# DataZooDE/anofox-statistics

Measured on AMD Instinct MI355X. Metric: group_fits_per_sec, higher is better.
Workload: dtype f64; 1 GPU; ols_fit_agg: 1000000 groups x n=1000 x p=8, device-resident grouped columns, fit_intercept=true, compute_inference=false; groups_total=1000000, groups_per_gpu=1000000, rows_per_group=1000, features=8, partition=contiguous key ranges over 1 rank(s); all-gather of 14-double records

## Files before the change

anofox-statistics_amd/csrc/accumulate_narrow.hip:

```cpp
#include <stdlib.h>

#include "common.h"
#include "wave_reduce.h"

namespace anofox {

typedef double dbl2u __attribute__((ext_vector_type(2), aligned(8)));

#ifndef ANOFOX_NARROW_NT
#define ANOFOX_NARROW_NT false
#endif
template <bool NT>
__device__ __forceinline__ dbl2u load2(const double *p) {
	if (NT) return __builtin_nontemporal_load(reinterpret_cast<const dbl2u *>(p));
	return *reinterpret_cast<const dbl2u *>(p);
}

template <int Z>
struct NarrowTile {
	double n0[Z], n1[Z], nw0, nw1;
};

template <int P, bool WEIGHTED>
__device__ __forceinline__ void narrow_load_tile(const BatchArgs &args, int64_t base, int64_t hi, int lane, NarrowTile<P + 1> &t) {
	const int64_t r0 = base + 2 * lane;
	if (base + 128 <= hi) {
#pragma unroll
		for (int j = 0; j < P; ++j) {
			const dbl2u v = load2<ANOFOX_NARROW_NT>(args.x[j] + r0);
			t.n0[j] = v.x;
			t.n1[j] = v.y;
		}
		{
			const dbl2u v = load2<ANOFOX_NARROW_NT>(args.y + r0);
			t.n0[P] = v.x;
			t.n1[P] = v.y;
		}
		if (WEIGHTED) {
			const dbl2u v = load2<ANOFOX_NARROW_NT>(args.w + r0);
			t.nw0 = v.x;
			t.nw1 = v.y;
		}
	} else {
		const int64_t c0 = r0 < hi ? r0 : hi - 1, c1 = r0 + 1 < hi ? r0 + 1 : hi - 1;
#pragma unroll
		for (int j = 0; j < P; ++j) {
			t.n0[j] = args.x[j][c0];
			t.n1[j] = args.x[j][c1];
		}
		t.n0[P] = args.y[c0];
		t.n1[P] = args.y[c1];
		if (WEIGHTED) {
			t.nw0 = args.w[c0];
			t.nw1 = args.w[c1];
// ... 114 lines not shown
	for (int k = 0; k < ZZ; ++k) v[L::OFF_Q + k] = c.q[k];
	v[L::OFF_SW] = c.sw;

	transpose_reduce64(v, lane);

	if (lane < L::KRED) rec[lane] = v[0];

	double e = 0.0;
#pragma unroll
	for (int a = 0; a < Z; ++a) e = (lane == a) ? c.first[a] : e;
	e = (lane == Z) ? (double)c.cnt : e;
	e = (lane == Z + 1) ? (double)c.mask : e;
	if (lane < Z + 2) rec[L::KRED + lane] = e;
}

template <int P, bool WEIGHTED, bool CENTER, bool PREFETCH>
__device__ __forceinline__ void accumulate_rows(const BatchArgs &args, int64_t lo, int64_t hi, double *rec, int lane) {
	constexpr int Z = P + 1;
	NarrowAcc<P> c;
	narrow_acc_init<P>(c);
	NarrowTile<Z> t;
	if (PREFETCH && lo < hi) narrow_load_tile<P, WEIGHTED>(args, lo, hi, lane, t);
	for (int64_t base = lo; base < hi; base += 128) {
		if (!PREFETCH) narrow_load_tile<P, WEIGHTED>(args, base, hi, lane, t);
		double z0[Z], z1[Z];
		double w0 = 1.0, w1 = 1.0;
#pragma unroll
		for (int a = 0; a < Z; ++a) {
			z0[a] = t.n0[a];
			z1[a] = t.n1[a];
		}
		if (WEIGHTED) {
			w0 = t.nw0;
			w1 = t.nw1;
		}
		if (PREFETCH && base + 128 < hi) narrow_load_tile<P, WEIGHTED>(args, base + 128, hi, lane, t);
		narrow_tile_compute<P, WEIGHTED, CENTER>(c, z0, z1, w0, w1, base + 2 * lane, hi);
	}
	narrow_acc_finish<P, CENTER>(c, rec, lane);
}

__device__ __forceinline__ SegHeader *seg_header(void *t) { return static_cast<SegHeader *>(t); }
__device__ __forceinline__ SegBigGroup *seg_big(void *t) { return reinterpret_cast<SegBigGroup *>(seg_header(t) + 1); }
__device__ __forceinline__ SegEntry *seg_entries(void *t) { return reinterpret_cast<SegEntry *>(seg_big(t) + kSegMaxBig); }
__device__ __forceinline__ double *seg_records(void *t) { return reinterpret_cast<double *>(seg_entries(t) + kSegMaxSegments); }

__device__ __forceinline__ bool narrow_register_big_group(const BatchArgs &args, int64_t g, int64_t lo, int64_t hi, int lane) {
	{
		SegHeader *h = seg_header(args.seg_table);
		const int64_t S = args.seg_rows;
		const int nseg = (int)((hi - lo + S - 1) / S);
// ... 21 lines not shown
			if (slot >= 0) return true;
		}
	}
	return false;
}

template <int P, bool WEIGHTED, bool CENTER, bool PF>
__device__ __forceinline__ void accumulate_group(const BatchArgs &args, int64_t g, int lane) {
	using L = MomentLayout<P>;
	const int64_t lo = args.row_offsets[g];
	const int64_t hi = group_row_end(args, g);
	if (args.seg_table && hi - lo > args.seg_rows && narrow_register_big_group(args, g, lo, hi, lane)) return;
	accumulate_rows<P, WEIGHTED, CENTER, PF>(args, lo, hi, args.moments + g * (int64_t)L::REC, lane);
}

template <int P, bool WEIGHTED, bool CENTER, bool PF>
__global__ __launch_bounds__(256) void accumulate_narrow_kernel(BatchArgs args) {
	const int lane = threadIdx.x & 63;
	const int64_t g = __builtin_amdgcn_readfirstlane((int)(threadIdx.x >> 6)) + (int64_t)blockIdx.x * 4;
	if (g >= args.n_groups) return;
	accumulate_group<P, WEIGHTED, CENTER, PF>(args, g, lane);
}

template <int P, bool WEIGHTED, bool CENTER, bool PF>
__global__ __launch_bounds__(256) void accumulate_narrow_list_kernel(BatchArgs args, const int32_t *list, const int32_t *count) {
	const int lane = threadIdx.x & 63;
	const int n = *count;
	const int n_waves = (int)gridDim.x * 4;
	for (int v = (int)blockIdx.x * 4 + __builtin_amdgcn_readfirstlane((int)(threadIdx.x >> 6)); v < n; v += n_waves)
		accumulate_group<P, WEIGHTED, CENTER, PF>(args, list[v], lane);
}

template <int P, bool CENTER>
__device__ void merge_segments(const double *seg_rec, int nseg, double *rec, int lane) {
// ... 54 lines not shown
	if (v >= total) return;
	const SegEntry e = seg_entries(args.seg_table)[v];
	if (e.slot < 0) return;
	double *recs = seg_records(args.seg_table);
	accumulate_rows<P, WEIGHTED, CENTER, PF>(args, e.lo, e.hi, recs + (int64_t)v * L::REC, lane);
	__threadfence();
	SegBigGroup *b = seg_big(args.seg_table) + e.slot;
	int old = 0;
	if (lane == 0) old = atomicAdd(&b->done, 1);
	old = __builtin_amdgcn_readfirstlane(old);
	if (old != b->nseg - 1) return;
	__threadfence();
	merge_segments<P, CENTER>(recs + (int64_t)b->base * L::REC, b->nseg, args.moments + b->g * (int64_t)L::REC, lane);
}

template <int P, bool PF>
static hipError_t launch_pn(const BatchArgs &a, hipStream_t stream) {
	const dim3 block(256);
	const dim3 grid((unsigned)((a.n_groups + 3) / 4));
	const dim3 seg_grid((unsigned)((kSegMaxSegments + 3) / 4));
	const bool weighted = a.model == ANOFOX_HIP_MODEL_WLS;
	const bool center = a.fit_intercept != 0;
#define ANOFOX_ACC_LAUNCH(W, C)                                                                               \
	do {                                                                                                      \
		hipLaunchKernelGGL((accumulate_narrow_kernel<P, W, C, PF>), grid, block, 0, stream, a);               \
		if (a.seg_table) hipLaunchKernelGGL((accumulate_segments_kernel<P, W, C, PF>), seg_grid, block, 0, stream, a); \
	} while (0)
	if (weighted) {
		if (center) ANOFOX_ACC_LAUNCH(true, true);
		else ANOFOX_ACC_LAUNCH(true, false);
	} else {
		if (center) ANOFOX_ACC_LAUNCH(false, true);
		else ANOFOX_ACC_LAUNCH(false, false);
	}
#undef ANOFOX_ACC_LAUNCH
	return hipGetLastError();
}

template <int P, bool PF>
static hipError_t launch_list_pn(const BatchArgs &a, const int32_t *list, const int32_t *count, hipStream_t stream) {
	const dim3 block(256), grid(2048);
	const dim3 seg_grid((unsigned)((kSegMaxSegments + 3) / 4));
	const bool weighted = a.model == ANOFOX_HIP_MODEL_WLS;
	const bool center = a.fit_intercept != 0;
#define ANOFOX_ACC_LIST_LAUNCH(W, C)                                                                          \
	do {                                                                                                      \
		hipLaunchKernelGGL((accumulate_narrow_list_kernel<P, W, C, PF>), grid, block, 0, stream, a, list, count); \
		if (a.seg_table) hipLaunchKernelGGL((accumulate_segments_kernel<P, W, C, PF>), seg_grid, block, 0, stream, a); \
	} while (0)
	if (weighted) {
		if (center) ANOFOX_ACC_LIST_LAUNCH(true, true);
		else ANOFOX_ACC_LIST_LAUNCH(true, false);
	} else {
		if (center) ANOFOX_ACC_LIST_LAUNCH(false, true);
		else ANOFOX_ACC_LIST_LAUNCH(false, false);
	}
#undef ANOFOX_ACC_LIST_LAUNCH
	return hipGetLastError();
}

template <int P>
static hipError_t launch_p(const BatchArgs &a, const int32_t *list, const int32_t *count, hipStream_t stream) {
	static const int pf = [] { const char *e = getenv("ANOFOX_ACC_PF"); return e ? atoi(e) : 1; }();
	if (list) return pf ? launch_list_pn<P, true>(a, list, count, stream) : launch_list_pn<P, false>(a, list, count, stream);
	return pf ? launch_pn<P, true>(a, stream) : launch_pn<P, false>(a, stream);
}

static hipError_t launch_any(const BatchArgs &a, const int32_t *list, const int32_t *count, hipStream_t stream) {
	if (a.n_groups <= 0) return hipSuccess;
	switch (a.p) {
	case 1: return launch_p<1>(a, list, count, stream);
	case 2: return launch_p<2>(a, list, count, stream);
	case 3: return launch_p<3>(a, list, count, stream);
	case 4: return launch_p<4>(a, list, count, stream);
	case 5: return launch_p<5>(a, list, count, stream);
	case 6: return launch_p<6>(a, list, count, stream);
	case 7: return launch_p<7>(a, list, count, stream);
	case 8: return launch_p<8>(a, list, count, stream);
	default: return hipErrorInvalidValue;
	}
}

hipError_t launch_accumulate_narrow(const BatchArgs &a, hipStream_t stream) { return launch_any(a, nullptr, nullptr, stream); }

hipError_t launch_accumulate_narrow_list(const BatchArgs &a, const int32_t *list, const int32_t *count, hipStream_t stream) {
	return launch_any(a, list, count, stream);
}

}
```

anofox-statistics_amd/csrc/common.h:

```cpp
#pragma once
#include <hip/hip_runtime.h>
#include <stdint.h>

#include "../../include/anofox_stats_hip.h"

namespace anofox {

constexpr int kNarrowMaxP = 8;

constexpr size_t kTcritTableBytes = 4096;

template <int P>
struct MomentLayout {
	static constexpr int Z = P + 1;
	static constexpr int ZZ = Z * (Z + 1) / 2;
	static constexpr int OFF_S = 0;
	static constexpr int OFF_Q = Z;
	static constexpr int OFF_SW = Z + ZZ;
	static constexpr int KRED = Z + ZZ + 1;
	static constexpr int OFF_FIRST = KRED;
	static constexpr int OFF_CNT = KRED + Z;
	static constexpr int OFF_MASK = KRED + Z + 1;
	static constexpr int REC = KRED + Z + 2;
	__host__ __device__ static constexpr int q_index(int a, int b) {
// ... 29 lines not shown
	int lambda_scaling;
	int hc_type;
	double confidence_level;
	double alpha;
	double *moments;
	double *core;
	double *inference;
	int32_t *refine_list;
	int32_t *refine_count;
	double *refine_vec;
	void *tcrit_table;
	const int64_t *rule_counts;
	void *seg_table;
	int64_t seg_rows;
	const int64_t *row_ends;
};
inline __host__ __device__ int64_t group_row_end(const BatchArgs &a, int64_t g) { return a.row_ends ? a.row_ends[g] : a.row_offsets[g + 1]; }

constexpr int kSegTargetWaves = 2048;
constexpr int kSegMaxBig = kSegTargetWaves + 8;
constexpr int kSegMaxSegments = 2 * kSegTargetWaves + 16;
constexpr int64_t kSegMinRows = 8192;
struct SegHeader {
	int32_t seg_total;
	int32_t big_total;
	int32_t pad[14];
};
struct SegBigGroup {
	int64_t g;
	int32_t base;
	int32_t nseg;
// ... 384 lines not shown
```

anofox-statistics_amd/csrc/host_api.hip:

```cpp
#include <math.h>
#include <stdio.h>
#include <stdlib.h>
#include <string.h>

#include <memory>
#include <mutex>
#include <string>
#include <vector>

#include "common.h"
#include "host_math.h"

using namespace anofox;

#include "context.h"

using namespace anofox::host;

namespace {

struct Workspace {
	void *seg_table;
	double *moments;
	double *refine_vec;
// ... 35 lines not shown
	}
	if (hip_fail(launch_residual_grad_wide(a, ss), "wide residual kernel launch", e)) return false;
	if (hip_fail(solve(2), "wide final kernel launch", e)) return false;
	if (!mid && hip_fail(launch_inference_wide_finish(a, ss), "wide inference finish kernel launch", e)) return false;
	if (a.hc_type != ANOFOX_HC_NONE && a.inference && a.model != ANOFOX_HIP_MODEL_RIDGE) {
		if (!ensure_buffer(&ctx->aux, &ctx->aux_bytes, (size_t)slab * sizeof(double), "hc scratch", e)) return false;
		a.hc_df = (double *)ctx->aux;
		if (hip_fail(launch_hc_wide(a, ss), "wide hc kernel launch", e)) return false;
	}
	static const bool refit_dd_on = !(getenv("ANOFOX_REFIT_DD") && atoi(getenv("ANOFOX_REFIT_DD")) == 0);
	if (refit_dd_on && hip_fail(launch_refit_dd_wide(a, ss), "double-double refit kernel launch", e)) return false;
	return true;
}

bool regression_narrow_stage(AnofoxHipContext *ctx, BatchArgs &a, hipStream_t st, void *, AnofoxError *e) {
	if (hip_fail(launch_solve_narrow(a, st), "solve kernel launch", e)) return false;
	if (hip_fail(launch_refine_fused_narrow(a, kRefineSteps, st), "refine kernel launch", e)) return false;
	if (a.hc_type != ANOFOX_HC_NONE && a.inference && a.model != ANOFOX_HIP_MODEL_RIDGE) {
		const size_t b_tab = align_up(sizeof(PredictSegTable), 256);
		if (!ensure_buffer(&ctx->aux, &ctx->aux_bytes, b_tab + hc_prep_bytes(a.n_groups, a.p), "hc scratch", e)) return false;
		if (hip_fail(hipMemsetAsync(ctx->aux, 0, 64, st), "hipMemsetAsync", e)) return false;
		if (hip_fail(launch_hc_narrow(a, (double *)((char *)ctx->aux + b_tab), ctx->aux, st), "hc kernel launch", e)) return false;
	}
	static const bool refit_dd_on = !(getenv("ANOFOX_REFIT_DD") && atoi(getenv("ANOFOX_REFIT_DD")) == 0);
	if (refit_dd_on && hip_fail(launch_refit_dd_narrow(a, st), "double-double refit kernel launch", e)) return false;
	return true;
}

const SolveStages kRegressionStages = {regression_narrow_stage, regression_wide_stage, nullptr};

bool run_wide_batch(AnofoxHipContext *ctx, int64_t G, size_t p, int64_t n_rows, const int64_t *d_off,
// ... 185 lines not shown
	hipEvent_t e0 = nullptr, e1 = nullptr, e2 = nullptr;
	if (ctx->timing) {
		e0 = get_event(ctx);
		e1 = get_event(ctx);
		e2 = get_event(ctx);
		(void)hipEventRecord(e0, st);
	}
	if (ctx->gate_wait) {
		hipEvent_t gw = ctx->gate_wait;
		ctx->gate_wait = nullptr;
		if (hip_fail(hipStreamWaitEvent(st, gw, 0), "hipStreamWaitEvent", e)) return false;
	}
	if (ctx->timing) (void)hipEventRecord(e0, st);
	static const bool small_on = !(getenv("ANOFOX_ACC_SMALL") && atoi(getenv("ANOFOX_ACC_SMALL")) == 0);
	const int segw = (small_on && !a.row_ends && n_rows > 0 && G < (int64_t)0x7fffffff) ? accumulate_small_segment_width((double)n_rows / (double)G) : 0;
	if (segw) {
		int32_t *big_count = ws.refine_count + 4;
		if (hip_fail(launch_accumulate_small(a, segw, ws.refine_list, big_count, st), "accumulate kernel launch", e)) return false;
		if (hip_fail(launch_accumulate_narrow_list(a, ws.refine_list, big_count, st), "accumulate kernel launch", e)) return false;
	} else if (hip_fail(launch_accumulate_narrow(a, st), "accumulate kernel launch", e)) {
		return false;
	}
	if (ctx->timing) (void)hipEventRecord(e1, st);
	if (ctx->gate_record) {
		hipEvent_t gr = ctx->gate_record;
		ctx->gate_record = nullptr;
		if (hip_fail(hipEventRecord(gr, st), "hipEventRecord", e)) return false;
	}
	if (!stages.narrow(ctx, a, st, stages.user, e)) return false;
	if (ctx->timing) {
// ... 1694 lines not shown
```

anofox-statistics_amd/csrc/solve_narrow.hip:

```cpp
#include "common.h"
#include "device_math.h"
#include "dd_arith.h"

namespace anofox {

static_assert(sizeof(TcritSlot) * kTcritSlots == kTcritTableBytes, "t memo does not fill its workspace slice");

namespace {

constexpr double kAliasTol = 1e-11;
constexpr double kAliasBand = 1e-13;
constexpr double kRefineTol = 1e-7;
constexpr double kPivotWarn = 1e-3;

__device__ __forceinline__ double nan64() { return __builtin_nan(""); }

enum { MODE_PRIMARY = 0, MODE_UPDATE = 1, MODE_FINAL = 2 };

template <int P, int MODE>
__device__ void solve_one(const BatchArgs &args, int64_t g) {
	using L = MomentLayout<P>;
	constexpr int Z = L::Z;
	const int p = P;
	const bool icpt = args.fit_intercept != 0;
	const int model = args.model;

	double *core = args.core + g * (int64_t)(p + 6);
	double *inf = (args.inference && args.compute_inference) ? args.inference + g * (int64_t)(5 * p + 2) : nullptr;
	const double *rv = args.refine_vec + g * (int64_t)refine_vec_len(p);

	int status = ANOFOX_ERROR_SUCCESS;
	double coef[P];
	double se[P], tv[P], pv[P], cl[P], cu[P];
#pragma unroll
	for (int j = 0; j < P; ++j) coef[j] = se[j] = tv[j] = pv[j] = cl[j] = cu[j] = nan64();
	double intercept = nan64(), r2 = nan64(), adj = nan64(), rse = nan64(), fstat = nan64(), fp = nan64();
	double nobs = nan64();
	bool has_inf = false;
	bool refine = false;

	const double *rec = args.moments + g * (int64_t)L::REC;
	const int64_t nrows = args.rule_counts ? args.rule_counts[g] : args.row_offsets[g + 1] - args.row_offsets[g];

	do {
		if (nrows < 2) { status = ANOFOX_HIP_STATUS_NULL_TOO_FEW_ROWS; break; }
		if (model == ANOFOX_HIP_MODEL_RIDGE && args.alpha < 0.0) { status = ANOFOX_ERROR_INVALID_ALPHA; break; }
		const double cnt = rec[L::OFF_CNT];
		if (!(cnt > 0.0)) { status = ANOFOX_ERROR_NO_VALID_DATA; break; }
		const double sw = rec[L::OFF_SW];
		const unsigned mask = (unsigned)rec[L::OFF_MASK];
		const int p_eff = __popc(mask);

		double s[Z], first[Z];
#pragma unroll
		for (int a = 0; a < Z; ++a) { s[a] = rec[L::OFF_S + a]; first[a] = rec[L::OFF_FIRST + a]; }
		const double qyy = rec[L::q_index(P, P)];
		const double cyy_centred = qyy - s[P] * s[P] / sw;
		const double ymean = (icpt ? first[P] : 0.0) + s[P] / sw;

		if (p_eff == 0) {
			if (!icpt) { status = ANOFOX_ERROR_INSUFFICIENT_DATA; break; }
			intercept = ymean;
			r2 = 0.0;
			adj = 0.0;
			rse = (model == ANOFOX_HIP_MODEL_WLS) ? sqrt(cyy_centred / sw) : sqrt(cyy_centred / (cnt - 1.0));
			nobs = cnt;
			break;
		}
		if (cnt < (double)(p_eff + (icpt ? 1 : 0))) { status = ANOFOX_ERROR_INSUFFICIENT_DATA; break; }

		double A[P][P];
		double c[P];
		bool active[P];
#pragma unroll
		for (int i = 0; i < P; ++i) {
			active[i] = (mask >> i) & 1u;
#pragma unroll
			for (int j = 0; j <= i; ++j) {
				const double qij = rec[L::q_index(j, i)];
				A[i][j] = icpt ? qij - s[i] * s[j] / sw : qij;
			}
			const double qiy = rec[L::q_index(i, P)];
			c[i] = icpt ? qiy - s[i] * s[P] / sw : qiy;
		}
		const double tss = icpt ? cyy_centred : qyy;

		double lam = 0.0, lam_rows = 0.0;
		bool glmnet_cancels = false;
		if (model == ANOFOX_HIP_MODEL_RIDGE) {
			lam = args.alpha;
			if (args.lambda_scaling == ANOFOX_LAMBDA_SCALING_GLMNET) {
				lam = cnt * args.alpha / sqrt(cyy_centred / cnt);
				glmnet_cancels = !icpt && !(cyy_centred * kGlmnetCancelRatio > qyy);
				if (MODE != MODE_PRIMARY && !icpt) lam_rows = cnt * args.alpha / sqrt(rv[p + 2] / cnt);
				else lam_rows = lam;
			} else {
				lam_rows = lam;
			}
#pragma unroll
			for (int i = 0; i < P; ++i) A[i][i] += (MODE == MODE_PRIMARY) ? lam : lam_rows;
		}

		double diag0[P];
#pragma unroll
		for (int j = 0; j < P; ++j) diag0[j] = A[j][j];
		double min_ratio = 1.0;
		bool band = false;
#pragma unroll
		for (int j = 0; j < P; ++j) {
			double d = A[j][j];
#pragma unroll
			for (int k = 0; k < j; ++k) d -= A[j][k] * A[j][k];
			const bool ok = active[j] && (d > kAliasTol * diag0[j]) && (d > 0.0);
			band = band || (active[j] && !ok && d > kAliasBand * diag0[j]);
			active[j] = ok;
			if (ok) min_ratio = fmin(min_ratio, d / diag0[j]);
			const double ljj = ok ? sqrt(d) : 1.0;
			A[j][j] = ljj;
			const double inv = 1.0 / ljj;
#pragma unroll
			for (int i = j + 1; i < P; ++i) {
				double t = A[i][j];
#pragma unroll
				for (int k = 0; k < j; ++k) t -= A[i][k] * A[j][k];
				A[i][j] = ok ? t * inv : 0.0;
			}
			if (!ok) {
#pragma unroll
				for (int k = 0; k < j; ++k) A[j][k] = 0.0;
			}
		}
		int rank = 0;
#pragma unroll
		for (int j = 0; j < P; ++j) rank += active[j] ? 1 : 0;

		auto solve_llt = [&](const double (&rhs)[P], double (&zf)[P], double (&x)[P]) {
#pragma unroll
			for (int i = 0; i < P; ++i) {
				double t = rhs[i];
#pragma unroll
				for (int k = 0; k < i; ++k) t -= A[i][k] * zf[k];
				zf[i] = active[i] ? t / A[i][i] : 0.0;
			}
#pragma unroll
			for (int i = P - 1; i >= 0; --i) {
				double t = zf[i];
#pragma unroll
				for (int k = i + 1; k < P; ++k) t -= A[k][i] * x[k];
				x[i] = active[i] ? t / A[i][i] : 0.0;
			}
		};

		double beta[P];
		double rss;
		if (MODE == MODE_PRIMARY) {
			double zf[P];
			solve_llt(c, zf, beta);
			double zz = 0.0, bc = 0.0, bb = 0.0;
#pragma unroll
			for (int i = 0; i < P; ++i) { zz += zf[i] * zf[i]; bc += beta[i] * c[i]; bb += beta[i] * beta[i]; }
			rss = (model == ANOFOX_HIP_MODEL_RIDGE) ? tss - bc - lam * bb : tss - zz;
			refine = !(rss > kRefineTol * tss) || (min_ratio < kPivotWarn) || glmnet_cancels || band;
			double bmax = 0.0;
#pragma unroll
			for (int i = 0; i < P; ++i) bmax = fmax(bmax, active[i] ? fabs(beta[i]) : 0.0);
#pragma unroll
			for (int i = 0; i < P; ++i) refine = refine || (active[i] && coef_bound_weak(beta[i], bmax, diag0[i], tss, min_ratio));
		} else {
#pragma unroll
			for (int i = 0; i < P; ++i) {
				const double b = core[i];
				beta[i] = active[i] ? b : 0.0;
			}
			rss = rv[0];
		}

		if (MODE == MODE_UPDATE) {
			const double gs = rv[1];
			double gc[P], u[P], delta[P];
#pragma unroll
			for (int i = 0; i < P; ++i) {
				double gi = rv[2 + i];
				if (icpt) gi -= (s[i] / sw) * gs;
				gc[i] = active[i] ? gi - lam_rows * beta[i] : 0.0;
			}
			solve_llt(gc, u, delta);
#pragma unroll
			for (int i = 0; i < P; ++i) beta[i] += delta[i];
		}

		const int n_par = rank + (icpt ? 1 : 0);
		const double df = cnt - (double)n_par;
		const double dfm = (double)rank;

		double b0 = 0.0;
		if (icpt) {
			b0 = ymean;
#pragma unroll
			for (int i = 0; i < P; ++i) b0 -= beta[i] * (first[i] + s[i] / sw);
			intercept = b0;
		}
#pragma unroll
		for (int i = 0; i < P; ++i) coef[i] = active[i] ? beta[i] : nan64();
		if (MODE == MODE_UPDATE) {
#pragma unroll
			for (int j = 0; j < P; ++j) core[j] = coef[j];
			core[p] = intercept;
			return;
		}
		r2 = 1.0 - rss / tss;
		adj = 1.0 - (1.0 - r2) * (cnt - (icpt ? 1.0 : 0.0)) / df;
		rse = sqrt(rss / df);
		nobs = cnt;
		fstat = ((tss - rss) / dfm) / (rss / df);

		if (inf) {
			has_inf = true;
			fp = dm_f_sf(fstat, dfm, df);
			const double sigma2 = rss / df;
			const double tcrit = dm_tcrit_cached(static_cast<TcritSlot *>(args.tcrit_table), 0.5 * (1.0 + args.confidence_level), df);
#pragma unroll
			for (int j = 0; j < P; ++j) {
				double wcol[P];
				double dj = 0.0;
#pragma unroll
				for (int i = j; i < P; ++i) {
					double t = (i == j) ? 1.0 : 0.0;
#pragma unroll
					for (int k = j; k < i; ++k) t -= A[i][k] * wcol[k];
					wcol[i] = active[i] ? t / A[i][i] : 0.0;
					dj += wcol[i] * wcol[i];
				}
				if (active[j]) {
					se[j] = sqrt(sigma2 * dj);
					tv[j] = beta[j] / se[j];
					pv[j] = dm_t_two_sided_p(tv[j], df);
					cl[j] = beta[j] - tcrit * se[j];
					cu[j] = beta[j] + tcrit * se[j];
				}
			}
		}
	} while (false);

	if (MODE == MODE_UPDATE) return;

	if (status != ANOFOX_ERROR_SUCCESS) {
#pragma unroll
		for (int j = 0; j < P; ++j) coef[j] = nan64();
		intercept = r2 = adj = rse = nobs = nan64();
	}
#pragma unroll
	for (int j = 0; j < P; ++j) core[j] = coef[j];
	core[p] = intercept;
	core[p + 1] = r2;
	core[p + 2] = adj;
	core[p + 3] = rse;
	core[p + 4] = nobs;
	core[p + 5] = (double)status;
	if (inf) {
		if (!has_inf) {
#pragma unroll
			for (int j = 0; j < P; ++j) se[j] = tv[j] = pv[j] = cl[j] = cu[j] = nan64();
			fstat = fp = nan64();
		}
#pragma unroll
		for (int j = 0; j < P; ++j) {
			inf[j] = se[j];
			inf[p + j] = tv[j];
			inf[2 * p + j] = pv[j];
			inf[3 * p + j] = cl[j];
			inf[4 * p + j] = cu[j];
		}
		inf[5 * p] = fstat;
		inf[5 * p + 1] = fp;
	}
	if (MODE == MODE_PRIMARY && refine && status == ANOFOX_ERROR_SUCCESS) {
		const int slot = atomicAdd(args.refine_count, 1);
		args.refine_list[slot] = (int32_t)g;
	}
}

template <int P>
__global__ __launch_bounds__(64) void solve_narrow_kernel(BatchArgs args) {
	const int64_t g = (int64_t)blockIdx.x * blockDim.x + threadIdx.x;
	if (g >= args.n_groups) return;
	solve_one<P, MODE_PRIMARY>(args, g);
}

__device__ __forceinline__ void residual_grad_wave(const BatchArgs &args, int64_t g, int lane) {
#pragma clang fp contract(off)
	const int p = args.p;
	const bool weighted = args.model == ANOFOX_HIP_MODEL_WLS;
	const int Z = p + 1;
	const int off_first = Z + Z * (Z + 1) / 2 + 1;
	const int rec_len = moment_record_len(p);
	const double *core = args.core + g * (int64_t)(p + 6);
	const double *rec = args.moments + g * (int64_t)rec_len;
	double b[kNarrowMaxP], sh[kNarrowMaxP], acc_h[kNarrowMaxP + 1], acc_l[kNarrowMaxP + 1];
	const double ybar = rec[p] / rec[Z + Z * (Z + 1) / 2] + (args.fit_intercept ? rec[off_first + p] : 0.0);
#pragma unroll
	for (int j = 0; j < kNarrowMaxP; ++j) {
// ... 53 lines not shown
	for (int k = 0; k < kNarrowMaxP + 1; ++k) mine = (lane == 1 + k) ? acc_h[k] + acc_l[k] : mine;
	if (lane == p + 2) mine = cyy;
	if (lane < p + 3) out[lane] = mine;
}

template <int P>
__global__ __launch_bounds__(64) void refine_fused_kernel(BatchArgs args, int steps) {
	const int lane = threadIdx.x & 63;
	const int n = *args.refine_count;
	for (int i = blockIdx.x; i < n; i += gridDim.x) {
		const int64_t g = args.refine_list[i];
		for (int it = 0; it <= steps; ++it) {
			residual_grad_wave(args, g, lane);
			__builtin_amdgcn_fence(__ATOMIC_SEQ_CST, "workgroup");
			if (lane == 0) {
				if (it < steps) solve_one<P, MODE_UPDATE>(args, g);
				else solve_one<P, MODE_FINAL>(args, g);
			}
			__builtin_amdgcn_fence(__ATOMIC_SEQ_CST, "workgroup");
		}
	}
}

template <int P>
hipError_t launch_solve_p(const BatchArgs &a, hipStream_t stream) {
	const unsigned grid = (unsigned)((a.n_groups + 63) / 64);
	hipLaunchKernelGGL((solve_narrow_kernel<P>), dim3(grid), dim3(64), 0, stream, a);
	return hipGetLastError();
}

}

// ... 39 lines not shown
```

Before: 80.60 million fits/s.

## Fuse narrow accumulation with primary solve, keeping moment records in LDS

Each wavefront now accumulates moments for up to 16 consecutive groups into shared memory. It then solves them in the same kernel, one lane per group, and writes only the core results plus the moments of groups queued for refinement. This removes the separate solve kernel launch and the global write and read of every group's moment record. Big segmented groups get a small dedicated solve kernel. The solve code moves into a shared header, and an env switch lets non-temporal loads be chosen at runtime. The tradeoff is that the serial per-lane solve runs inside the bandwidth-bound kernel, and the LDS use may cut occupancy.

```diff
diff --git a/anofox-statistics_amd/csrc/accumulate_narrow.hip b/anofox-statistics_amd/csrc/accumulate_narrow.hip
--- a/anofox-statistics_amd/csrc/accumulate_narrow.hip
+++ b/anofox-statistics_amd/csrc/accumulate_narrow.hip
@@ -1,15 +1,13 @@
 #include <stdlib.h>
 
 #include "common.h"
+#include "solve_narrow_impl.h"
 #include "wave_reduce.h"
 
 namespace anofox {
 
 typedef double dbl2u __attribute__((ext_vector_type(2), aligned(8)));
 
-#ifndef ANOFOX_NARROW_NT
-#define ANOFOX_NARROW_NT false
-#endif
 template <bool NT>
 __device__ __forceinline__ dbl2u load2(const double *p) {
 	if (NT) return __builtin_nontemporal_load(reinterpret_cast<const dbl2u *>(p));
@@ -21,23 +19,23 @@
 	double n0[Z], n1[Z], nw0, nw1;
 };
 
-template <int P, bool WEIGHTED>
+template <int P, bool WEIGHTED, bool NT>
 __device__ __forceinline__ void narrow_load_tile(const BatchArgs &args, int64_t base, int64_t hi, int lane, NarrowTile<P + 1> &t) {
 	const int64_t r0 = base + 2 * lane;
 	if (base + 128 <= hi) {
 #pragma unroll
 		for (int j = 0; j < P; ++j) {
-			const dbl2u v = load2<ANOFOX_NARROW_NT>(args.x[j] + r0);
+			const dbl2u v = load2<NT>(args.x[j] + r0);
 			t.n0[j] = v.x;
 			t.n1[j] = v.y;
 		}
 		{
-			const dbl2u v = load2<ANOFOX_NARROW_NT>(args.y + r0);
+			const dbl2u v = load2<NT>(args.y + r0);
 			t.n0[P] = v.x;
 			t.n1[P] = v.y;
 		}
 		if (WEIGHTED) {
-			const dbl2u v = load2<ANOFOX_NARROW_NT>(args.w + r0);
+			const dbl2u v = load2<NT>(args.w + r0);
 			t.nw0 = v.x;
 			t.nw1 = v.y;
 		}
@@ -182,15 +180,15 @@
 	if (lane < Z + 2) rec[L::KRED + lane] = e;
 }
 
-template <int P, bool WEIGHTED, bool CENTER, bool PREFETCH>
+template <int P, bool WEIGHTED, bool CENTER, bool PREFETCH, bool NT = false>
 __device__ __forceinline__ void accumulate_rows(const BatchArgs &args, int64_t lo, int64_t hi, double *rec, int lane) {
 	constexpr int Z = P + 1;
 	NarrowAcc<P> c;
 	narrow_acc_init<P>(c);
 	NarrowTile<Z> t;
-	if (PREFETCH && lo < hi) narrow_load_tile<P, WEIGHTED>(args, lo, hi, lane, t);
+	if (PREFETCH && lo < hi) narrow_load_tile<P, WEIGHTED, NT>(args, lo, hi, lane, t);
 	for (int64_t base = lo; base < hi; base += 128) {
-		if (!PREFETCH) narrow_load_tile<P, WEIGHTED>(args, base, hi, lane, t);
+		if (!PREFETCH) narrow_load_tile<P, WEIGHTED, NT>(args, base, hi, lane, t);
 		double z0[Z], z1[Z];
 		double w0 = 1.0, w1 = 1.0;
 #pragma unroll
@@ -202,7 +200,7 @@
 			w0 = t.nw0;
 			w1 = t.nw1;
 		}
-		if (PREFETCH && base + 128 < hi) narrow_load_tile<P, WEIGHTED>(args, base + 128, hi, lane, t);
+		if (PREFETCH && base + 128 < hi) narrow_load_tile<P, WEIGHTED, NT>(args, base + 128, hi, lane, t);
 		narrow_tile_compute<P, WEIGHTED, CENTER>(c, z0, z1, w0, w1, base + 2 * lane, hi);
 	}
 	narrow_acc_finish<P, CENTER>(c, rec, lane);
@@ -254,10 +252,55 @@
 	accumulate_rows<P, WEIGHTED, CENTER, PF>(args, lo, hi, args.moments + g * (int64_t)L::REC, lane);
 }
 
-template <int P, bool WEIGHTED, bool CENTER, bool PF>
-__global__ __launch_bounds__(256) void accumulate_narrow_kernel(BatchArgs args) {
+#ifndef ANOFOX_NARROW_FUSED_K
+#define ANOFOX_NARROW_FUSED_K 16
+#endif
+constexpr int kFusedGroups = ANOFOX_NARROW_FUSED_K;
+static_assert(kFusedGroups >= 1 && kFusedGroups <= 32, "groups per wavefront: one lane each, a 32-bit skip mask");
+
+template <int P, bool WEIGHTED, bool CENTER, bool PF, bool NT>
+__device__ __forceinline__ void accumulate_solve_groups(const BatchArgs &args, int64_t g0, int lane, double *lrec, double *lcore) {
+	using L = MomentLayout<P>;
+	constexpr int CL = P + 6;
+	const int n = (int)(args.n_groups - g0 < kFusedGroups ? args.n_groups - g0 : kFusedGroups);
+	unsigned skip = 0;
+	for (int i = 0; i < n; ++i) {
+		const int64_t g = g0 + i;
+		const int64_t lo = args.row_offsets[g];
+		const int64_t hi = group_row_end(args, g);
+		if (args.seg_table && hi - lo > args.seg_rows && narrow_register_big_group(args, g, lo, hi, lane)) {
+			skip |= 1u << i;
+			continue;
+		}
+		accumulate_rows<P, WEIGHTED, CENTER, PF, NT>(args, lo, hi, lrec + i * L::REC, lane);
+	}
+	__builtin_amdgcn_fence(__ATOMIC_SEQ_CST, "workgroup");
+	bool queued = false;
+	if (lane < n && !((skip >> lane) & 1u)) queued = solve_one<P, MODE_PRIMARY, false>(args, g0 + lane, lrec + lane * L::REC, lcore + lane * CL);
+	__builtin_amdgcn_fence(__ATOMIC_SEQ_CST, "workgroup");
+	double *core = args.core + g0 * CL;
+	for (int k = lane; k < n * CL; k += 64)
+		if (!((skip >> (k / CL)) & 1u)) core[k] = lcore[k];
+	for (unsigned long long q = __ballot(queued); q != 0ull; q &= q - 1ull) {
+		const int i = __ffsll((long long)q) - 1;
+		for (int k = lane; k < L::REC; k += 64) args.moments[(g0 + i) * L::REC + k] = lrec[i * L::REC + k];
+	}
+}
+
+template <int P, bool WEIGHTED, bool CENTER, bool PF, bool FUSED = false, bool NT = false>
+__global__ __launch_bounds__(256) __attribute__((amdgpu_waves_per_eu(FUSED ? 2 : 1))) void accumulate_narrow_kernel(BatchArgs args) {
 	const int lane = threadIdx.x & 63;
-	const int64_t g = __builtin_amdgcn_readfirstlane((int)(threadIdx.x >> 6)) + (int64_t)blockIdx.x * 4;
+	const int wave = __builtin_amdgcn_readfirstlane((int)(threadIdx.x >> 6));
+	if (FUSED) {
+		using L = MomentLayout<P>;
+		__shared__ double lrec[4][kFusedGroups * L::REC];
+		__shared__ double lcore[4][kFusedGroups * (P + 6)];
+		const int64_t g0 = ((int64_t)blockIdx.x * 4 + wave) * kFusedGroups;
+		if (g0 >= args.n_groups) return;
+		accumulate_solve_groups<P, WEIGHTED, CENTER, PF, NT>(args, g0, lane, lrec[wave], lcore[wave]);
+		return;
+	}
+	const int64_t g = wave + (int64_t)blockIdx.x * 4;
 	if (g >= args.n_groups) return;
 	accumulate_group<P, WEIGHTED, CENTER, PF>(args, g, lane);
 }
@@ -342,16 +385,28 @@
 	merge_segments<P, CENTER>(recs + (int64_t)b->base * L::REC, b->nseg, args.moments + b->g * (int64_t)L::REC, lane);
 }
 
-template <int P, bool PF>
+template <int P>
+__global__ __launch_bounds__(64) void solve_big_narrow_kernel(BatchArgs args) {
+	const int slot = (int)(blockIdx.x * blockDim.x + threadIdx.x);
+	const int total = seg_header(args.seg_table)->big_total;
+	if (slot >= total) return;
+	const int64_t g = seg_big(args.seg_table)[slot].g;
+	solve_one<P, MODE_PRIMARY>(args, g, args.moments + g * (int64_t)MomentLayout<P>::REC, args.core + g * (int64_t)(P + 6));
+}
+
+template <int P, bool PF, bool FUSED, bool NT>
 static hipError_t launch_pn(const BatchArgs &a, hipStream_t stream) {
 	const dim3 block(256);
-	const dim3 grid((unsigned)((a.n_groups + 3) / 4));
+	const int64_t per_block = FUSED ? 4 * kFusedGroups : 4;
+	const dim3 grid((unsigned)((a.n_groups + per_block - 1) / per_block));
 	const dim3 seg_grid((unsigned)((kSegMaxSegments + 3) / 4));
 	const bool weighted = a.model == ANOFOX_HIP_MODEL_WLS;
 	const bool center = a.fit_intercept != 0;
 #define ANOFOX_ACC_LAUNCH(W, C)                                                                               \
 	do {                                                                                                      \
-		hipLaunchKernelGGL((accumulate_narrow_kernel<P, W, C, PF>), grid, block, 0, stream, a);               \
+		constexpr bool F = FUSED && narrow_fused_fits(P, W, C);                                                      \
+		if (FUSED && !F) return hipErrorNotSupported;                                                         \
+		hipLaunchKernelGGL((accumulate_narrow_kernel<P, W, C, PF, F, F && NT>), grid, block, 0, stream, a);   \
 		if (a.seg_table) hipLaunchKernelGGL((accumulate_segments_kernel<P, W, C, PF>), seg_grid, block, 0, stream, a); \
 	} while (0)
 	if (weighted) {
@@ -362,6 +417,8 @@
 		else ANOFOX_ACC_LAUNCH(false, false);
 	}
 #undef ANOFOX_ACC_LAUNCH
+	if (FUSED && a.seg_table)
+		hipLaunchKernelGGL((solve_big_narrow_kernel<P>), dim3((unsigned)((kSegMaxBig + 63) / 64)), dim3(64), 0, stream, a);
 	return hipGetLastError();
 }
 
@@ -388,31 +445,36 @@
 }
 
 template <int P>
-static hipError_t launch_p(const BatchArgs &a, const int32_t *list, const int32_t *count, hipStream_t stream) {
+static hipError_t launch_p(const BatchArgs &a, const int32_t *list, const int32_t *count, bool fused, hipStream_t stream) {
 	static const int pf = [] { const char *e = getenv("ANOFOX_ACC_PF"); return e ? atoi(e) : 1; }();
+	static const int nt = [] { const char *e = getenv("ANOFOX_NARROW_NT"); return e ? atoi(e) : 0; }();
 	if (list) return pf ? launch_list_pn<P, true>(a, list, count, stream) : launch_list_pn<P, false>(a, list, count, stream);
-	return pf ? launch_pn<P, true>(a, stream) : launch_pn<P, false>(a, stream);
-}
-
-static hipError_t launch_any(const BatchArgs &a, const int32_t *list, const int32_t *count, hipStream_t stream) {
+	if (fused) {
+		if (!pf) return launch_pn<P, false, true, false>(a, stream);
+		return nt ? launch_pn<P, true, true, true>(a, stream) : launch_pn<P, true, true, false>(a, stream);
+	}
+	return pf ? launch_pn<P, true, false, false>(a, stream) : launch_pn<P, false, false, false>(a, stream);
+}
+
+static hipError_t launch_any(const BatchArgs &a, const int32_t *list, const int32_t *count, bool fused, hipStream_t stream) {
 	if (a.n_groups <= 0) return hipSuccess;
 	switch (a.p) {
-	case 1: return launch_p<1>(a, list, count, stream);
-	case 2: return launch_p<2>(a, list, count, stream);
-	case 3: return launch_p<3>(a, list, count, stream);
-	case 4: return launch_p<4>(a, list, count, stream);
-	case 5: return launch_p<5>(a, list, count, stream);
-	case 6: return launch_p<6>(a, list, count, stream);
-	case 7: return launch_p<7>(a, list, count, stream);
-	case 8: return launch_p<8>(a, list, count, stream);
+	case 1: return launch_p<1>(a, list, count, fused, stream);
+	case 2: return launch_p<2>(a, list, count, fused, stream);
+	case 3: return launch_p<3>(a, list, count, fused, stream);
+	case 4: return launch_p<4>(a, list, count, fused, stream);
+	case 5: return launch_p<5>(a, list, count, fused, stream);
+	case 6: return launch_p<6>(a, list, count, fused, stream);
+	case 7: return launch_p<7>(a, list, count, fused, stream);
+	case 8: return launch_p<8>(a, list, count, fused, stream);
 	default: return hipErrorInvalidValue;
 	}
 }
 
-hipError_t launch_accumulate_narrow(const BatchArgs &a, hipStream_t stream) { return launch_any(a, nullptr, nullptr, stream); }
+hipError_t launch_accumulate_narrow(const BatchArgs &a, hipStream_t stream) { return launch_any(a, nullptr, nullptr, a.primary_solved != 0, stream); }
 
 hipError_t launch_accumulate_narrow_list(const BatchArgs &a, const int32_t *list, const int32_t *count, hipStream_t stream) {
-	return launch_any(a, list, count, stream);
-}
-
-}
+	return launch_any(a, list, count, false, stream);
+}
+
+}
diff --git a/anofox-statistics_amd/csrc/common.h b/anofox-statistics_amd/csrc/common.h
--- a/anofox-statistics_amd/csrc/common.h
+++ b/anofox-statistics_amd/csrc/common.h
@@ -67,7 +67,11 @@
 	void *seg_table;
 	int64_t seg_rows;
 	const int64_t *row_ends;
-};
+	int primary_solved;
+};
+inline constexpr __host__ __device__ bool narrow_fused_fits(int p, bool weighted, bool center) {
+	return p >= 1 && p <= kNarrowMaxP && !(p == 8 && weighted && center);
+}
 inline __host__ __device__ int64_t group_row_end(const BatchArgs &a, int64_t g) { return a.row_ends ? a.row_ends[g] : a.row_offsets[g + 1]; }
 
 constexpr int kSegTargetWaves = 2048;
diff --git a/anofox-statistics_amd/csrc/host_api.hip b/anofox-statistics_amd/csrc/host_api.hip
--- a/anofox-statistics_amd/csrc/host_api.hip
+++ b/anofox-statistics_amd/csrc/host_api.hip
@@ -73,7 +73,7 @@
 }
 
 bool regression_narrow_stage(AnofoxHipContext *ctx, BatchArgs &a, hipStream_t st, void *, AnofoxError *e) {
-	if (hip_fail(launch_solve_narrow(a, st), "solve kernel launch", e)) return false;
+	if (!a.primary_solved && hip_fail(launch_solve_narrow(a, st), "solve kernel launch", e)) return false;
 	if (hip_fail(launch_refine_fused_narrow(a, kRefineSteps, st), "refine kernel launch", e)) return false;
 	if (a.hc_type != ANOFOX_HC_NONE && a.inference && a.model != ANOFOX_HIP_MODEL_RIDGE) {
 		const size_t b_tab = align_up(sizeof(PredictSegTable), 256);
@@ -289,6 +289,9 @@
 	if (ctx->timing) (void)hipEventRecord(e0, st);
 	static const bool small_on = !(getenv("ANOFOX_ACC_SMALL") && atoi(getenv("ANOFOX_ACC_SMALL")) == 0);
 	const int segw = (small_on && !a.row_ends && n_rows > 0 && G < (int64_t)0x7fffffff) ? accumulate_small_segment_width((double)n_rows / (double)G) : 0;
+	static const bool fused_on = !(getenv("ANOFOX_NARROW_FUSED") && atoi(getenv("ANOFOX_NARROW_FUSED")) == 0);
+	a.primary_solved = (fused_on && stages.narrow == regression_narrow_stage && !a.row_ends && !segw && !a.inference &&
+	                    narrow_fused_fits(a.p, a.model == ANOFOX_HIP_MODEL_WLS, a.fit_intercept != 0)) ? 1 : 0;
 	if (segw) {
 		int32_t *big_count = ws.refine_count + 4;
 		if (hip_fail(launch_accumulate_small(a, segw, ws.refine_list, big_count, st), "accumulate kernel launch", e)) return false;
diff --git a/anofox-statistics_amd/csrc/solve_narrow.hip b/anofox-statistics_amd/csrc/solve_narrow.hip
--- a/anofox-statistics_amd/csrc/solve_narrow.hip
+++ b/anofox-statistics_amd/csrc/solve_narrow.hip
@@ -1,6 +1,7 @@
 #include "common.h"
 #include "device_math.h"
 #include "dd_arith.h"
+#include "solve_narrow_impl.h"
 
 namespace anofox {
 
@@ -8,283 +9,11 @@
 
 namespace {
 
-constexpr double kAliasTol = 1e-11;
-constexpr double kAliasBand = 1e-13;
-constexpr double kRefineTol = 1e-7;
-constexpr double kPivotWarn = 1e-3;
-
-__device__ __forceinline__ double nan64() { return __builtin_nan(""); }
-
-enum { MODE_PRIMARY = 0, MODE_UPDATE = 1, MODE_FINAL = 2 };
-
-template <int P, int MODE>
-__device__ void solve_one(const BatchArgs &args, int64_t g) {
-	using L = MomentLayout<P>;
-	constexpr int Z = L::Z;
-	const int p = P;
-	const bool icpt = args.fit_intercept != 0;
-	const int model = args.model;
-
-	double *core = args.core + g * (int64_t)(p + 6);
-	double *inf = (args.inference && args.compute_inference) ? args.inference + g * (int64_t)(5 * p + 2) : nullptr;
-	const double *rv = args.refine_vec + g * (int64_t)refine_vec_len(p);
-
-	int status = ANOFOX_ERROR_SUCCESS;
-	double coef[P];
-	double se[P], tv[P], pv[P], cl[P], cu[P];
-#pragma unroll
-	for (int j = 0; j < P; ++j) coef[j] = se[j] = tv[j] = pv[j] = cl[j] = cu[j] = nan64();
-	double intercept = nan64(), r2 = nan64(), adj = nan64(), rse = nan64(), fstat = nan64(), fp = nan64();
-	double nobs = nan64();
-	bool has_inf = false;
-	bool refine = false;
-
-	const double *rec = args.moments + g * (int64_t)L::REC;
-	const int64_t nrows = args.rule_counts ? args.rule_counts[g] : args.row_offsets[g + 1] - args.row_offsets[g];
-
-	do {
-		if (nrows < 2) { status = ANOFOX_HIP_STATUS_NULL_TOO_FEW_ROWS; break; }
-		if (model == ANOFOX_HIP_MODEL_RIDGE && args.alpha < 0.0) { status = ANOFOX_ERROR_INVALID_ALPHA; break; }
-		const double cnt = rec[L::OFF_CNT];
-		if (!(cnt > 0.0)) { status = ANOFOX_ERROR_NO_VALID_DATA; break; }
-		const double sw = rec[L::OFF_SW];
-		const unsigned mask = (unsigned)rec[L::OFF_MASK];
-		const int p_eff = __popc(mask);
-
-		double s[Z], first[Z];
-#pragma unroll
-		for (int a = 0; a < Z; ++a) { s[a] = rec[L::OFF_S + a]; first[a] = rec[L::OFF_FIRST + a]; }
-		const double qyy = rec[L::q_index(P, P)];
-		const double cyy_centred = qyy - s[P] * s[P] / sw;
-		const double ymean = (icpt ? first[P] : 0.0) + s[P] / sw;
-
-		if (p_eff == 0) {
-			if (!icpt) { status = ANOFOX_ERROR_INSUFFICIENT_DATA; break; }
-			intercept = ymean;
-			r2 = 0.0;
-			adj = 0.0;
-			rse = (model == ANOFOX_HIP_MODEL_WLS) ? sqrt(cyy_centred / sw) : sqrt(cyy_centred / (cnt - 1.0));
-			nobs = cnt;
-			break;
-		}
-		if (cnt < (double)(p_eff + (icpt ? 1 : 0))) { status = ANOFOX_ERROR_INSUFFICIENT_DATA; break; }
-
-		double A[P][P];
-		double c[P];
-		bool active[P];
-#pragma unroll
-		for (int i = 0; i < P; ++i) {
-			active[i] = (mask >> i) & 1u;
-#pragma unroll
-			for (int j = 0; j <= i; ++j) {
-				const double qij = rec[L::q_index(j, i)];
-				A[i][j] = icpt ? qij - s[i] * s[j] / sw : qij;
-			}
-			const double qiy = rec[L::q_index(i, P)];
-			c[i] = icpt ? qiy - s[i] * s[P] / sw : qiy;
-		}
-		const double tss = icpt ? cyy_centred : qyy;
-
-		double lam = 0.0, lam_rows = 0.0;
-		bool glmnet_cancels = false;
-		if (model == ANOFOX_HIP_MODEL_RIDGE) {
-			lam = args.alpha;
-			if (args.lambda_scaling == ANOFOX_LAMBDA_SCALING_GLMNET) {
-				lam = cnt * args.alpha / sqrt(cyy_centred / cnt);
-				glmnet_cancels = !icpt && !(cyy_centred * kGlmnetCancelRatio > qyy);
-				if (MODE != MODE_PRIMARY && !icpt) lam_rows = cnt * args.alpha / sqrt(rv[p + 2] / cnt);
-				else lam_rows = lam;
-			} else {
-				lam_rows = lam;
-			}
-#pragma unroll
-			for (int i = 0; i < P; ++i) A[i][i] += (MODE == MODE_PRIMARY) ? lam : lam_rows;
-		}
-
-		double diag0[P];
-#pragma unroll
-		for (int j = 0; j < P; ++j) diag0[j] = A[j][j];
-		double min_ratio = 1.0;
-		bool band = false;
-#pragma unroll
-		for (int j = 0; j < P; ++j) {
-			double d = A[j][j];
-#pragma unroll
-			for (int k = 0; k < j; ++k) d -= A[j][k] * A[j][k];
-			const bool ok = active[j] && (d > kAliasTol * diag0[j]) && (d > 0.0);
-			band = band || (active[j] && !ok && d > kAliasBand * diag0[j]);
-			active[j] = ok;
-			if (ok) min_ratio = fmin(min_ratio, d / diag0[j]);
-			const double ljj = ok ? sqrt(d) : 1.0;
-			A[j][j] = ljj;
-			const double inv = 1.0 / ljj;
-#pragma unroll
-			for (int i = j + 1; i < P; ++i) {
-				double t = A[i][j];
-#pragma unroll
-				for (int k = 0; k < j; ++k) t -= A[i][k] * A[j][k];
-				A[i][j] = ok ? t * inv : 0.0;
-			}
-			if (!ok) {
-#pragma unroll
-				for (int k = 0; k < j; ++k) A[j][k] = 0.0;
-			}
-		}
-		int rank = 0;
-#pragma unroll
-		for (int j = 0; j < P; ++j) rank += active[j] ? 1 : 0;
-
-		auto solve_llt = [&](const double (&rhs)[P], double (&zf)[P], double (&x)[P]) {
-#pragma unroll
-			for (int i = 0; i < P; ++i) {
-				double t = rhs[i];
-#pragma unroll
-				for (int k = 0; k < i; ++k) t -= A[i][k] * zf[k];
-				zf[i] = active[i] ? t / A[i][i] : 0.0;
-			}
-#pragma unroll
-			for (int i = P - 1; i >= 0; --i) {
-				double t = zf[i];
-#pragma unroll
-				for (int k = i + 1; k < P; ++k) t -= A[k][i] * x[k];
-				x[i] = active[i] ? t / A[i][i] : 0.0;
-			}
-		};
-
-		double beta[P];
-		double rss;
-		if (MODE == MODE_PRIMARY) {
-			double zf[P];
-			solve_llt(c, zf, beta);
-			double zz = 0.0, bc = 0.0, bb = 0.0;
-#pragma unroll
-			for (int i = 0; i < P; ++i) { zz += zf[i] * zf[i]; bc += beta[i] * c[i]; bb += beta[i] * beta[i]; }
-			rss = (model == ANOFOX_HIP_MODEL_RIDGE) ? tss - bc - lam * bb : tss - zz;
-			refine = !(rss > kRefineTol * tss) || (min_ratio < kPivotWarn) || glmnet_cancels || band;
-			double bmax = 0.0;
-#pragma unroll
-			for (int i = 0; i < P; ++i) bmax = fmax(bmax, active[i] ? fabs(beta[i]) : 0.0);
-#pragma unroll
-			for (int i = 0; i < P; ++i) refine = refine || (active[i] && coef_bound_weak(beta[i], bmax, diag0[i], tss, min_ratio));
-		} else {
-#pragma unroll
-			for (int i = 0; i < P; ++i) {
-				const double b = core[i];
-				beta[i] = active[i] ? b : 0.0;
-			}
-			rss = rv[0];
-		}
-
-		if (MODE == MODE_UPDATE) {
-			const double gs = rv[1];
-			double gc[P], u[P], delta[P];
-#pragma unroll
-			for (int i = 0; i < P; ++i) {
-				double gi = rv[2 + i];
-				if (icpt) gi -= (s[i] / sw) * gs;
-				gc[i] = active[i] ? gi - lam_rows * beta[i] : 0.0;
-			}
-			solve_llt(gc, u, delta);
-#pragma unroll
-			for (int i = 0; i < P; ++i) beta[i] += delta[i];
-		}
-
-		const int n_par = rank + (icpt ? 1 : 0);
-		const double df = cnt - (double)n_par;
-		const double dfm = (double)rank;
-
-		double b0 = 0.0;
-		if (icpt) {
-			b0 = ymean;
-#pragma unroll
-			for (int i = 0; i < P; ++i) b0 -= beta[i] * (first[i] + s[i] / sw);
-			intercept = b0;
-		}
-#pragma unroll
-		for (int i = 0; i < P; ++i) coef[i] = active[i] ? beta[i] : nan64();
-		if (MODE == MODE_UPDATE) {
-#pragma unroll
-			for (int j = 0; j < P; ++j) core[j] = coef[j];
-			core[p] = intercept;
-			return;
-		}
-		r2 = 1.0 - rss / tss;
-		adj = 1.0 - (1.0 - r2) * (cnt - (icpt ? 1.0 : 0.0)) / df;
-		rse = sqrt(rss / df);
-		nobs = cnt;
-		fstat = ((tss - rss) / dfm) / (rss / df);
-
-		if (inf) {
-			has_inf = true;
-			fp = dm_f_sf(fstat, dfm, df);
-			const double sigma2 = rss / df;
-			const double tcrit = dm_tcrit_cached(static_cast<TcritSlot *>(args.tcrit_table), 0.5 * (1.0 + args.confidence_level), df);
-#pragma unroll
-			for (int j = 0; j < P; ++j) {
-				double wcol[P];
-				double dj = 0.0;
-#pragma unroll
-				for (int i = j; i < P; ++i) {
-					double t = (i == j) ? 1.0 : 0.0;
-#pragma unroll
-					for (int k = j; k < i; ++k) t -= A[i][k] * wcol[k];
-					wcol[i] = active[i] ? t / A[i][i] : 0.0;
-					dj += wcol[i] * wcol[i];
-				}
-				if (active[j]) {
-					se[j] = sqrt(sigma2 * dj);
-					tv[j] = beta[j] / se[j];
-					pv[j] = dm_t_two_sided_p(tv[j], df);
-					cl[j] = beta[j] - tcrit * se[j];
-					cu[j] = beta[j] + tcrit * se[j];
-				}
-			}
-		}
-	} while (false);
-
-	if (MODE == MODE_UPDATE) return;
-
-	if (status != ANOFOX_ERROR_SUCCESS) {
-#pragma unroll
-		for (int j = 0; j < P; ++j) coef[j] = nan64();
-		intercept = r2 = adj = rse = nobs = nan64();
-	}
-#pragma unroll
-	for (int j = 0; j < P; ++j) core[j] = coef[j];
-	core[p] = intercept;
-	core[p + 1] = r2;
-	core[p + 2] = adj;
-	core[p + 3] = rse;
-	core[p + 4] = nobs;
-	core[p + 5] = (double)status;
-	if (inf) {
-		if (!has_inf) {
-#pragma unroll
-			for (int j = 0; j < P; ++j) se[j] = tv[j] = pv[j] = cl[j] = cu[j] = nan64();
-			fstat = fp = nan64();
-		}
-#pragma unroll
-		for (int j = 0; j < P; ++j) {
-			inf[j] = se[j];
-			inf[p + j] = tv[j];
-			inf[2 * p + j] = pv[j];
-			inf[3 * p + j] = cl[j];
-			inf[4 * p + j] = cu[j];
-		}
-		inf[5 * p] = fstat;
-		inf[5 * p + 1] = fp;
-	}
-	if (MODE == MODE_PRIMARY && refine && status == ANOFOX_ERROR_SUCCESS) {
-		const int slot = atomicAdd(args.refine_count, 1);
-		args.refine_list[slot] = (int32_t)g;
-	}
-}
-
 template <int P>
 __global__ __launch_bounds__(64) void solve_narrow_kernel(BatchArgs args) {
 	const int64_t g = (int64_t)blockIdx.x * blockDim.x + threadIdx.x;
 	if (g >= args.n_groups) return;
-	solve_one<P, MODE_PRIMARY>(args, g);
+	solve_one<P, MODE_PRIMARY>(args, g, args.moments + g * (int64_t)MomentLayout<P>::REC, args.core + g * (int64_t)(P + 6));
 }
 
 __device__ __forceinline__ void residual_grad_wave(const BatchArgs &args, int64_t g, int lane) {
@@ -368,8 +97,10 @@
 			residual_grad_wave(args, g, lane);
 			__builtin_amdgcn_fence(__ATOMIC_SEQ_CST, "workgroup");
 			if (lane == 0) {
-				if (it < steps) solve_one<P, MODE_UPDATE>(args, g);
-				else solve_one<P, MODE_FINAL>(args, g);
+				const double *rec = args.moments + g * (int64_t)MomentLayout<P>::REC;
+				double *core = args.core + g * (int64_t)(P + 6);
+				if (it < steps) solve_one<P, MODE_UPDATE>(args, g, rec, core);
+				else solve_one<P, MODE_FINAL>(args, g, rec, core);
 			}
 			__builtin_amdgcn_fence(__ATOMIC_SEQ_CST, "workgroup");
 		}
diff --git a/anofox-statistics_amd/csrc/solve_narrow_impl.h b/anofox-statistics_amd/csrc/solve_narrow_impl.h
--- /dev/null
+++ b/anofox-statistics_amd/csrc/solve_narrow_impl.h
@@ -0,0 +1,276 @@
+#pragma once
+
+#include "common.h"
+#include "device_math.h"
+
+namespace anofox {
+namespace {
+
+constexpr double kAliasTol = 1e-11;
+constexpr double kAliasBand = 1e-13;
+constexpr double kRefineTol = 1e-7;
+constexpr double kPivotWarn = 1e-3;
+
+__device__ __forceinline__ double nan64() { return __builtin_nan(""); }
+
+enum { MODE_PRIMARY = 0, MODE_UPDATE = 1, MODE_FINAL = 2 };
+
+template <int P, int MODE, bool INF = true>
+__device__ bool solve_one(const BatchArgs &args, int64_t g, const double *rec, double *core) {
+	using L = MomentLayout<P>;
+	constexpr int Z = L::Z;
+	const int p = P;
+	const bool icpt = args.fit_intercept != 0;
+	const int model = args.model;
+
+	double *inf = (INF && args.inference && args.compute_inference) ? args.inference + g * (int64_t)(5 * p + 2) : nullptr;
+	const double *rv = args.refine_vec + g * (int64_t)refine_vec_len(p);
+
+	int status = ANOFOX_ERROR_SUCCESS;
+	double coef[P];
+#pragma unroll
+	for (int j = 0; j < P; ++j) coef[j] = nan64();
+	double intercept = nan64(), r2 = nan64(), adj = nan64(), rse = nan64(), fstat = nan64(), fp = nan64();
+	double nobs = nan64();
+	bool has_inf = false;
+	bool refine = false;
+
+	const int64_t nrows = args.rule_counts ? args.rule_counts[g] : args.row_offsets[g + 1] - args.row_offsets[g];
+
+	do {
+		if (nrows < 2) { status = ANOFOX_HIP_STATUS_NULL_TOO_FEW_ROWS; break; }
+		if (model == ANOFOX_HIP_MODEL_RIDGE && args.alpha < 0.0) { status = ANOFOX_ERROR_INVALID_ALPHA; break; }
+		const double cnt = rec[L::OFF_CNT];
+		if (!(cnt > 0.0)) { status = ANOFOX_ERROR_NO_VALID_DATA; break; }
+		const double sw = rec[L::OFF_SW];
+		const unsigned mask = (unsigned)rec[L::OFF_MASK];
+		const int p_eff = __popc(mask);
+
+		double s[Z], first[Z];
+#pragma unroll
+		for (int a = 0; a < Z; ++a) { s[a] = rec[L::OFF_S + a]; first[a] = rec[L::OFF_FIRST + a]; }
+		const double qyy = rec[L::q_index(P, P)];
+		const double cyy_centred = qyy - s[P] * s[P] / sw;
+		const double ymean = (icpt ? first[P] : 0.0) + s[P] / sw;
+
+		if (p_eff == 0) {
+			if (!icpt) { status = ANOFOX_ERROR_INSUFFICIENT_DATA; break; }
+			intercept = ymean;
+			r2 = 0.0;
+			adj = 0.0;
+			rse = (model == ANOFOX_HIP_MODEL_WLS) ? sqrt(cyy_centred / sw) : sqrt(cyy_centred / (cnt - 1.0));
+			nobs = cnt;
+			break;
+		}
+		if (cnt < (double)(p_eff + (icpt ? 1 : 0))) { status = ANOFOX_ERROR_INSUFFICIENT_DATA; break; }
+
+		double A[P][P];
+		double c[P];
+		bool active[P];
+#pragma unroll
+		for (int i = 0; i < P; ++i) {
+			active[i] = (mask >> i) & 1u;
+#pragma unroll
+			for (int j = 0; j <= i; ++j) {
+				const double qij = rec[L::q_index(j, i)];
+				A[i][j] = icpt ? qij - s[i] * s[j] / sw : qij;
+			}
+			const double qiy = rec[L::q_index(i, P)];
+			c[i] = icpt ? qiy - s[i] * s[P] / sw : qiy;
+		}
+		const double tss = icpt ? cyy_centred : qyy;
+
+		double lam = 0.0, lam_rows = 0.0;
+		bool glmnet_cancels = false;
+		if (model == ANOFOX_HIP_MODEL_RIDGE) {
+			lam = args.alpha;
+			if (args.lambda_scaling == ANOFOX_LAMBDA_SCALING_GLMNET) {
+				lam = cnt * args.alpha / sqrt(cyy_centred / cnt);
+				glmnet_cancels = !icpt && !(cyy_centred * kGlmnetCancelRatio > qyy);
+				if (MODE != MODE_PRIMARY && !icpt) lam_rows = cnt * args.alpha / sqrt(rv[p + 2] / cnt);
+				else lam_rows = lam;
+			} else {
+				lam_rows = lam;
+			}
+#pragma unroll
+			for (int i = 0; i < P; ++i) A[i][i] += (MODE == MODE_PRIMARY) ? lam : lam_rows;
+		}
+
+		double diag0[P];
+#pragma unroll
+		for (int j = 0; j < P; ++j) diag0[j] = A[j][j];
+		double min_ratio = 1.0;
+		bool band = false;
+#pragma unroll
+		for (int j = 0; j < P; ++j) {
+			double d = A[j][j];
+#pragma unroll
+			for (int k = 0; k < j; ++k) d -= A[j][k] * A[j][k];
+			const bool ok = active[j] && (d > kAliasTol * diag0[j]) && (d > 0.0);
+			band = band || (active[j] && !ok && d > kAliasBand * diag0[j]);
+			active[j] = ok;
+			if (ok) min_ratio = fmin(min_ratio, d / diag0[j]);
+			const double ljj = ok ? sqrt(d) : 1.0;
+			A[j][j] = ljj;
+			const double inv = 1.0 / ljj;
+#pragma unroll
+			for (int i = j + 1; i < P; ++i) {
+				double t = A[i][j];
+#pragma unroll
+				for (int k = 0; k < j; ++k) t -= A[i][k] * A[j][k];
+				A[i][j] = ok ? t * inv : 0.0;
+			}
+			if (!ok) {
+#pragma unroll
+				for (int k = 0; k < j; ++k) A[j][k] = 0.0;
+			}
+		}
+		int rank = 0;
+#pragma unroll
+		for (int j = 0; j < P; ++j) rank += active[j] ? 1 : 0;
+
+		auto solve_llt = [&](const double (&rhs)[P], double (&zf)[P], double (&x)[P]) {
+#pragma unroll
+			for (int i = 0; i < P; ++i) {
+				double t = rhs[i];
+#pragma unroll
+				for (int k = 0; k < i; ++k) t -= A[i][k] * zf[k];
+				zf[i] = active[i] ? t / A[i][i] : 0.0;
+			}
+#pragma unroll
+			for (int i = P - 1; i >= 0; --i) {
+				double t = zf[i];
+#pragma unroll
+				for (int k = i + 1; k < P; ++k) t -= A[k][i] * x[k];
+				x[i] = active[i] ? t / A[i][i] : 0.0;
+			}
+		};
+
+		double beta[P];
+		double rss;
+		if (MODE == MODE_PRIMARY) {
+			double zf[P];
+			solve_llt(c, zf, beta);
+			double zz = 0.0, bc = 0.0, bb = 0.0;
+#pragma unroll
+			for (int i = 0; i < P; ++i) { zz += zf[i] * zf[i]; bc += beta[i] * c[i]; bb += beta[i] * beta[i]; }
+			rss = (model == ANOFOX_HIP_MODEL_RIDGE) ? tss - bc - lam * bb : tss - zz;
+			refine = !(rss > kRefineTol * tss) || (min_ratio < kPivotWarn) || glmnet_cancels || band;
+			double bmax = 0.0;
+#pragma unroll
+			for (int i = 0; i < P; ++i) bmax = fmax(bmax, active[i] ? fabs(beta[i]) : 0.0);
+#pragma unroll
+			for (int i = 0; i < P; ++i) refine = refine || (active[i] && coef_bound_weak(beta[i], bmax, diag0[i], tss, min_ratio));
+		} else {
+#pragma unroll
+			for (int i = 0; i < P; ++i) {
+				const double b = core[i];
+				beta[i] = active[i] ? b : 0.0;
+			}
+			rss = rv[0];
+		}
+
+		if (MODE == MODE_UPDATE) {
+			const double gs = rv[1];
+			double gc[P], u[P], delta[P];
+#pragma unroll
+			for (int i = 0; i < P; ++i) {
+				double gi = rv[2 + i];
+				if (icpt) gi -= (s[i] / sw) * gs;
+				gc[i] = active[i] ? gi - lam_rows * beta[i] : 0.0;
+			}
+			solve_llt(gc, u, delta);
+#pragma unroll
+			for (int i = 0; i < P; ++i) beta[i] += delta[i];
+		}
+
+		const int n_par = rank + (icpt ? 1 : 0);
+		const double df = cnt - (double)n_par;
+		const double dfm = (double)rank;
+
+		double b0 = 0.0;
+		if (icpt) {
+			b0 = ymean;
+#pragma unroll
+			for (int i = 0; i < P; ++i) b0 -= beta[i] * (first[i] + s[i] / sw);
+			intercept = b0;
+		}
+#pragma unroll
+		for (int i = 0; i < P; ++i) coef[i] = active[i] ? beta[i] : nan64();
+		if (MODE == MODE_UPDATE) {
+#pragma unroll
+			for (int j = 0; j < P; ++j) core[j] = coef[j];
+			core[p] = intercept;
+			return false;
+		}
+		r2 = 1.0 - rss / tss;
+		adj = 1.0 - (1.0 - r2) * (cnt - (icpt ? 1.0 : 0.0)) / df;
+		rse = sqrt(rss / df);
+		nobs = cnt;
+		fstat = ((tss - rss) / dfm) / (rss / df);
+
+		if (inf) {
+			has_inf = true;
+			fp = dm_f_sf(fstat, dfm, df);
+			const double sigma2 = rss / df;
+			const double tcrit = dm_tcrit_cached(static_cast<TcritSlot *>(args.tcrit_table), 0.5 * (1.0 + args.confidence_level), df);
+#pragma unroll
+			for (int j = 0; j < P; ++j) {
+				double wcol[P];
+				double dj = 0.0;
+#pragma unroll
+				for (int i = j; i < P; ++i) {
+					double t = (i == j) ? 1.0 : 0.0;
+#pragma unroll
+					for (int k = j; k < i; ++k) t -= A[i][k] * wcol[k];
+					wcol[i] = active[i] ? t / A[i][i] : 0.0;
+					dj += wcol[i] * wcol[i];
+				}
+				double se = nan64(), tv = nan64(), pv = nan64(), cl = nan64(), cu = nan64();
+				if (active[j]) {
+					se = sqrt(sigma2 * dj);
+					tv = beta[j] / se;
+					pv = dm_t_two_sided_p(tv, df);
+					cl = beta[j] - tcrit * se;
+					cu = beta[j] + tcrit * se;
+				}
+				inf[j] = se;
+				inf[p + j] = tv;
+				inf[2 * p + j] = pv;
+				inf[3 * p + j] = cl;
+				inf[4 * p + j] = cu;
+			}
+			inf[5 * p] = fstat;
+			inf[5 * p + 1] = fp;
+		}
+	} while (false);
+
+	if (MODE == MODE_UPDATE) return false;
+
+	if (status != ANOFOX_ERROR_SUCCESS) {
+#pragma unroll
+		for (int j = 0; j < P; ++j) coef[j] = nan64();
+		intercept = r2 = adj = rse = nobs = nan64();
+	}
+#pragma unroll
+	for (int j = 0; j < P; ++j) core[j] = coef[j];
+	core[p] = intercept;
+	core[p + 1] = r2;
+	core[p + 2] = adj;
+	core[p + 3] = rse;
+	core[p + 4] = nobs;
+	core[p + 5] = (double)status;
+	if (inf && !has_inf) {
+#pragma unroll
+		for (int k = 0; k < 5 * P + 2; ++k) inf[k] = nan64();
+	}
+	if (MODE == MODE_PRIMARY && refine && status == ANOFOX_ERROR_SUCCESS) {
+		const int slot = atomicAdd(args.refine_count, 1);
+		args.refine_list[slot] = (int32_t)g;
+		return true;
+	}
+	return false;
+}
+
+}
+}
```

Result: faster. 85.20 million fits/s, median of 6 (+5.7%).
